# bioinfomaticsCSU/deepsignal

Hardware: AMD Instinct MI355X
Metric: CpG sites/sec (batch=512, k=17, sig=360) (higher is better)
Workload: dtype f32; 1 GPU; configs[1]: 1xMI355X, batch=512, random-init CpG model weights, synthetic (17,360) features, fp32; batch=512, kmer_len=17, signal_len=360

## Files before the change

### deepsignal_amd/csrc/ds_kernels.hip

```cpp
#include "ds_device.h"

namespace ds {


template <int MT, int NT, int WM, int WN, int EPI, int AMODE, int BD, int KS, bool BF = false>
__global__ __launch_bounds__(64 * WM * WN, 1) void gemm_kernel(const GemmLaunch* __restrict__ L)
{
    static_assert(KS == 1, "the in-workgroup K split is retired (profiles/EXPERIMENTS.md)");
    constexpr int BM = WM * MT * 32;
    constexpr int LDA = KC + 4;
    constexpr int NTHR = 64 * WM * WN;
    constexpr int SLOTS = (BM * 4 + NTHR - 1) / NTHR;
    __shared__ __attribute__((aligned(16))) float smem_[2 * BM * LDA];

    const int lane = threadIdx.x & 63, wave_all = __builtin_amdgcn_readfirstlane(threadIdx.x >> 6);
    const int kl = wave_all / (WM * WN);
    const int wave = wave_all % (WM * WN);
    const int tid = threadIdx.x - kl * NTHR;
    float* const As0 = smem_ + kl * BM * LDA;
    float* const As1 = smem_ + (1 + kl) * BM * LDA;
    const int wm = wave % WM, wn = wave / WM;
    int bid;
    {
        const int total = L->total_tiles, q = total >> 3, r = total & 7;
// ... 525 lines not shown
    for (int nt = 0; nt < NT; ++nt) {
        cp[nt] = make_float4(0.f, 0.f, 0.f, 0.f);
        if (!C.c_zero) cp[nt] = gload4(C.c + mt_off + (unsigned)(((ng * 2 + nj) * NT + nt)) * 256 + lane4);
    }

#pragma unroll
    for (int nt = 0; nt < NT; ++nt) {
        asm volatile("" : "+v"(cp[nt].x), "+v"(cp[nt].y), "+v"(cp[nt].z), "+v"(cp[nt].w));
        asm volatile("" : "+v"(acc[nt]));
    }
    DS_LSTAMP(2, __builtin_amdgcn_s_memtime());
    const float* const fa0 = ring + mi * 256 + lane4;
    const float* const fb0 = ring + (2 + nj * NT) * 256 + lane4;
    auto stage = [&](int st, auto slot_c) __attribute__((always_inline)) {
        constexpr int SLOT = decltype(slot_c)::value;
        if (st + 1 < nstages) asm volatile("s_waitcnt vmcnt(%0)" ::"n"(LPS) : "memory");
        else asm volatile("s_waitcnt vmcnt(0)" ::: "memory");
        __builtin_amdgcn_s_barrier();
        if (st + 2 < nstages) request(st + 2, (SLOT + 2) % 3);
#pragma unroll
        for (int kgi = 0; kgi < KGS; ++kgi) {
            const float4 a = *reinterpret_cast<const float4*>(fa0 + SLOT * STAGE + kgi * FR * 256);
#pragma unroll
            for (int nt = 0; nt < NT; ++nt) {
                const float4 b = *reinterpret_cast<const float4*>(fb0 + SLOT * STAGE + (kgi * FR + nt) * 256);
                acc[nt] = __builtin_amdgcn_mfma_f32_32x32x2f32(b.x, a.x, acc[nt], 0, 0, 0);
                acc[nt] = __builtin_amdgcn_mfma_f32_32x32x2f32(b.y, a.y, acc[nt], 0, 0, 0);
                acc[nt] = __builtin_amdgcn_mfma_f32_32x32x2f32(b.z, a.z, acc[nt], 0, 0, 0);
                acc[nt] = __builtin_amdgcn_mfma_f32_32x32x2f32(b.w, a.w, acc[nt], 0, 0, 0);
            }
        }
    };
    for (int st = 0; st < nstages;) {
        stage(st, LdsSlot<0>{}); if (++st >= nstages) break;
        stage(st, LdsSlot<1>{}); if (++st >= nstages) break;
        stage(st, LdsSlot<2>{}); ++st;
    }

    DS_LSTAMP(3, __builtin_amdgcn_s_memtime());
    if (!valid) return;
#pragma unroll
    for (int nt = 0; nt < NT; ++nt) {
        const int ntile = (ng * 2 + nj) * NT + nt;
        float4 cn, hn;
        lstm_gates(acc[nt], cp[nt], cn, hn);
        const size_t off = mt_off + (unsigned)ntile * 256 + lane4;
        const v4f co = {cn.x, cn.y, cn.z, cn.w}, ho = {hn.x, hn.y, hn.z, hn.w};
        *(__attribute__((address_space(1))) v4f*)(C.c + off) = co;
        *(__attribute__((address_space(1))) v4f*)(C.h_out + off) = ho;
        if (C.h_row && row < n)
            *(__attribute__((address_space(1))) v4f*)(C.h_row + (size_t)row * 256 + ntile * 8 + 4 * half) = ho;
    }
    DS_LSTAMP(4, __builtin_amdgcn_s_memtime());
    DS_LSTAMP(5, __builtin_amdgcn_s_memrealtime());
#undef DS_LSTAMP
}

constexpr int LSTM_MT_BYTES_BF16 = 32 * 256 * 2;
template <int MTW, int NTW>
__global__ __launch_bounds__(256, MTW * NTW >= 4 ? 2 : 3) void lstm_cell_bf16_kernel(const LstmLaunch L_)
{
    const LstmLaunch* const Lp = &L_;
    constexpr int FRA = 2 * MTW, FRB = 2 * NTW, FR = FRA + FRB;
    constexpr int KGS = 2;
    constexpr int NF = KGS * FR;
    static_assert(NF % 4 == 0, "fragments of a stage are dealt to four waves");
    constexpr int LPS = NF / 4;
    constexpr int STAGE = NF * 256;
    extern __shared__ __attribute__((aligned(16))) float ring[];

    const int lane = threadIdx.x & 63, wave = __builtin_amdgcn_readfirstlane(threadIdx.x >> 6);
    const int mi = wave & 1, nj = wave >> 1;
    unsigned long long* const sdst = (Lp->dbg && blockIdx.x < DBG_MAX_WGS) ? Lp->dbg + (size_t)blockIdx.x * 8 : nullptr;
    const bool stamp = sdst != nullptr && threadIdx.x == 0;
#define DS_LSTAMP(i, v) do { if (stamp) sdst[i] = (v); } while (0)
    DS_LSTAMP(0, __builtin_amdgcn_s_memrealtime());
    DS_LSTAMP(1, __builtin_amdgcn_s_memtime());
    DS_LSTAMP(6, (unsigned long long)__builtin_amdgcn_s_getreg(63492));
    DS_LSTAMP(7, (unsigned long long)__builtin_amdgcn_s_getreg(63508));
    const int bid = lstm_logical_tile(blockIdx.x, gridDim.x, Lp->cls_tiles[0], Lp->cls_tiles[1]);
    const int mtiles = Lp->mtiles;
    const int mblocks = (mtiles + FRA - 1) / FRA;
    constexpr int NGROUPS = 32 / FRB;
    const int per_cell = mblocks * NGROUPS;
    const int ci = bid / per_cell, rem = bid - ci * per_cell;
    const int ng = rem % NGROUPS, mb = rem / NGROUPS;
    const LstmCell& C = Lp->cell[ci];
    const int half = lane >> 5, r31 = lane & 31;
    const int n = Lp->n, T = Lp->T;
    const unsigned lane16 = (unsigned)lane * 16, lane4 = (unsigned)lane * 4;

    const bool has_x = C.ax != nullptr, has_h = C.ah != nullptr;
    const int KS = (has_x ? 16 : 0) + (has_h ? 16 : 0);
    const int nstages = KS / KGS;
    const char* const a0 = reinterpret_cast<const char*>(has_x ? C.ax : C.ah);
    const long dseg = (has_x && has_h) ? (reinterpret_cast<const char*>(C.ah) - reinterpret_cast<const char*>(C.ax)) - 16 * 1024 : 0;
    const char* src[LPS];
    int kgi_[LPS];
    bool is_a[LPS];
#pragma unroll
    for (int j = 0; j < LPS; ++j) {
        const int q = wave + 4 * j, kgi = q / FR, f = q - kgi * FR;
        kgi_[j] = kgi;
        is_a[j] = f < FRA;
        if (f < FRA) {
            const int m = min(mb * FRA + f, mtiles - 1);
            src[j] = a0 + (size_t)m * LSTM_MT_BYTES_BF16 + (size_t)kgi * 1024;
        } else {
            const int ntile = ng * FRB + (f - FRA);
            src[j] = reinterpret_cast<const char*>(C.Bp) + ((size_t)ntile * C.kg_stride + kgi) * 1024;
        }
    }
    const unsigned ring_lds = (unsigned)(size_t)(__attribute__((address_space(3))) float*)ring;
    auto request = [&](int st, int slot) __attribute__((always_inline)) {
        const unsigned dst = __builtin_amdgcn_readfirstlane(ring_lds + (slot * STAGE + wave * 256) * 4);
#pragma unroll
        for (int j = 0; j < LPS; ++j) {
            const int ks = st * KGS + kgi_[j];
            const long off = (long)st * (KGS * 1024) + ((is_a[j] && ks >= 16) ? dseg : 0);
            glds16s(src[j] + off, lane16, dst + j * 4096);
        }
    };
    if (nstages > 0) request(0, 0);
    if (nstages > 1) request(1, 1);

    int mt[MTW];
    bool valid[MTW];
#pragma unroll
    for (int i = 0; i < MTW; ++i) {
        const int raw = mb * FRA + mi * MTW + i;
        valid[i] = raw < mtiles;
        mt[i] = valid[i] ? raw : mtiles - 1;
    }
    floatx16 acc[MTW][NTW];
    float4 cp[MTW][NTW];
#pragma unroll
    for (int i = 0; i < MTW; ++i) {
        const int row = mt[i] * 32 + r31;
        const int rowc = row < n ? row : n - 1;
#pragma unroll
        for (int j = 0; j < NTW; ++j) lstm_acc_init(C, (ng * FRB + nj * NTW + j) * 8 + 4 * half, rowc, T, acc[i][j]);
    }
    const bool c_zero = C.c_zero != 0;
#pragma unroll
    for (int i = 0; i < MTW; ++i)
#pragma unroll
        for (int j = 0; j < NTW; ++j) {
            cp[i][j] = make_float4(0.f, 0.f, 0.f, 0.f);
            if (!c_zero) cp[i][j] = gload4(C.c + (size_t)mt[i] * LSTM_MT_FLOATS + (unsigned)(ng * FRB + nj * NTW + j) * 256 + lane4);
        }
#pragma unroll
    for (int i = 0; i < MTW; ++i)
#pragma unroll
        for (int j = 0; j < NTW; ++j) {
            asm volatile("" : "+v"(cp[i][j].x), "+v"(cp[i][j].y), "+v"(cp[i][j].z), "+v"(cp[i][j].w));
            asm volatile("" : "+v"(acc[i][j]));
        }
    DS_LSTAMP(2, __builtin_amdgcn_s_memtime());

    const float* const fa0 = ring + (mi * MTW) * 256 + lane4;
    const float* const fb0 = ring + (FRA + nj * NTW) * 256 + lane4;
    auto stage = [&](int st, auto slot_c) __attribute__((always_inline)) {
        constexpr int SLOT = decltype(slot_c)::value;
        if (st + 1 < nstages) asm volatile("s_waitcnt vmcnt(%0)" ::"n"(LPS) : "memory");
        else asm volatile("s_waitcnt vmcnt(0)" ::: "memory");
        __builtin_amdgcn_s_barrier();
        if (st + 2 < nstages) request(st + 2, (SLOT + 2) % 3);
#pragma unroll
        for (int kgi = 0; kgi < KGS; ++kgi) {
            float4 a[MTW], b[NTW];
#pragma unroll
            for (int i = 0; i < MTW; ++i) a[i] = *reinterpret_cast<const float4*>(fa0 + SLOT * STAGE + (kgi * FR + i) * 256);
#pragma unroll
            for (int j = 0; j < NTW; ++j) b[j] = *reinterpret_cast<const float4*>(fb0 + SLOT * STAGE + (kgi * FR + j) * 256);
#pragma unroll
            for (int i = 0; i < MTW; ++i)
#pragma unroll
                for (int j = 0; j < NTW; ++j) acc[i][j] = mfma_bf_early(b[j], a[i], acc[i][j]);
        }
    };
    for (int st = 0; st < nstages;) {
        stage(st, LdsSlot<0>{}); if (++st >= nstages) break;
        stage(st, LdsSlot<1>{}); if (++st >= nstages) break;
        stage(st, LdsSlot<2>{}); ++st;
    }
    DS_LSTAMP(3, __builtin_amdgcn_s_memtime());

    typedef unsigned int u2v __attribute__((ext_vector_type(2)));
#pragma unroll
    for (int i = 0; i < MTW; ++i) {
        if (!valid[i]) continue;
        const int row = mt[i] * 32 + r31;
#pragma unroll
        for (int j = 0; j < NTW; ++j) {
            const int ntile = ng * FRB + nj * NTW + j;
            float4 cn, hn;
            lstm_gates(acc[i][j], cp[i][j], cn, hn);
            const v4f co = {cn.x, cn.y, cn.z, cn.w};
            *(__attribute__((address_space(1))) v4f*)(C.c + (size_t)mt[i] * LSTM_MT_FLOATS + (unsigned)ntile * 256 + lane4) = co;
            const u2v ho = {pack_bf2(hn.x, hn.y), pack_bf2(hn.z, hn.w)};
            char* const hb = reinterpret_cast<char*>(C.h_out) + (size_t)mt[i] * LSTM_MT_BYTES_BF16 + (unsigned)(ntile >> 1) * 1024 +
                             (unsigned)(((ntile & 1) * 32 + r31) * 16 + half * 8);
            *(__attribute__((address_space(1))) u2v*)hb = ho;
            if (C.h_row && row < n) {
                const v4f hr = {hn.x, hn.y, hn.z, hn.w};
                *(__attribute__((address_space(1))) v4f*)(C.h_row + (size_t)row * 256 + ntile * 8 + 4 * half) = hr;
            }
        }
    }
    DS_LSTAMP(4, __builtin_amdgcn_s_memtime());
    DS_LSTAMP(5, __builtin_amdgcn_s_memrealtime());
#undef DS_LSTAMP
}

hipError_t launch_lstm_cells(LstmTile tile, const LstmLaunch& L, hipStream_t s)
{
    if (L.ncell <= 0 || L.mtiles <= 0) return hipSuccess;
    const dim3 grid(L.ncell * lstm_tiles_per_cell(tile, L.mtiles));
    switch (tile) {
    case LT_LDS1: hipLaunchKernelGGL(lstm_cell_lds_kernel<1>, grid, dim3(256), 3 * 1 * 4 * 1024, s, L); break;
    case LT_LDS2: hipLaunchKernelGGL(lstm_cell_lds_kernel<2>, grid, dim3(256), 3 * 2 * 6 * 1024, s, L); break;
    case LT_B11: hipLaunchKernelGGL((lstm_cell_bf16_kernel<1, 1>), grid, dim3(256), 3 * 2 * 4 * 1024, s, L); break;
    case LT_B12: hipLaunchKernelGGL((lstm_cell_bf16_kernel<1, 2>), grid, dim3(256), 3 * 2 * 6 * 1024, s, L); break;
    case LT_B22: hipLaunchKernelGGL((lstm_cell_bf16_kernel<2, 2>), grid, dim3(256), 3 * 2 * 8 * 1024, s, L); break;
    case LT_F1: hipLaunchKernelGGL(lstm_cell_kernel<1>, grid, dim3(256), 0, s, L); break;
    case LT_F4: hipLaunchKernelGGL(lstm_cell_kernel<4>, grid, dim3(256), 0, s, L); break;
    case LT_S11: case LT_S12: case LT_S22: case LT_S28: case LT_COUNT: return hipErrorInvalidValue;
    }
    return hipGetLastError();
}

#ifndef DS_FUSED_WPS
#define DS_FUSED_WPS 2
#endif
#ifndef DS_FUSED_BD
#define DS_FUSED_BD 2
#endif
#ifndef DS_FUSED_POOLPRIO
#define DS_FUSED_POOLPRIO 0
#endif
#ifndef DS_FUSED_VD
#define DS_FUSED_VD 2
#endif
constexpr int F_LDA = KC + 4;
constexpr int F_LD1 = 100;
constexpr int F_LD2 = 68;

size_t inception_fused_lds_bytes(int tm, int W, int spt)
{
    const int tr32 = tm * 32;
    return (size_t)(tr32 * F_LD1 + (spt * (W + 4) + 5) * F_LD1 + tr32 * F_LD2 + tr32 + 192) * sizeof(float);
}

__device__ __forceinline__ void fused_unit_prefetch(const float* __restrict__ Bp, int ntaps, int nt, int lane, float4 (&ub)[20])
{
    const float* bsrc = Bp + ((size_t)(nt * ntaps * 4) * 64 + lane) * 4;
#pragma unroll
    for (int g = 0; g < 20; ++g)
        if (g < ntaps * 4) ub[g] = gload4(bsrc + g * 256);
}

template <int NTAPS>
__device__ __forceinline__ void fused_conv_unit(const float* T1, int rm, int coloff, int lane, const float4 (&ub)[20], floatx16& acc)
{
    const float* base = T1 + rm * F_LD1 + coloff + (lane >> 5) * 4;
#pragma unroll
    for (int t = 0; t < NTAPS; ++t) {
        const float* arow = base + (t - NTAPS / 2) * F_LD1;
#pragma unroll
        for (int g = 0; g < 4; ++g) {
            const float4 a = *reinterpret_cast<const float4*>(arow + g * 8);
            acc = __builtin_amdgcn_mfma_f32_32x32x2f32(ub[t * 4 + g].x, a.x, acc, 0, 0, 0);
            acc = __builtin_amdgcn_mfma_f32_32x32x2f32(ub[t * 4 + g].y, a.y, acc, 0, 0, 0);
            acc = __builtin_amdgcn_mfma_f32_32x32x2f32(ub[t * 4 + g].z, a.z, acc, 0, 0, 0);
            acc = __builtin_amdgcn_mfma_f32_32x32x2f32(ub[t * 4 + g].w, a.w, acc, 0, 0, 0);
        }
    }
}

struct FusedTagT { static constexpr bool value = true; };
struct FusedTagF { static constexpr bool value = false; };

template <int TM>
__device__ __forceinline__ void inception_fused_body(const FusedChain& c)
{
    constexpr int TR32 = TM * 32;
    extern __shared__ __attribute__((aligned(16))) float smem[];
    float* Ad = smem;
    float* Ys = smem;
    float* T1 = smem + TR32 * F_LD1;
    const int W = c.m[0].W, spt = c.m[0].spt;
    float* T2 = T1 + (spt * (W + 4) + 5) * F_LD1;
    int* rowmap = reinterpret_cast<int*>(T2 + TR32 * F_LD2);
    float* const Bs = reinterpret_cast<float*>(rowmap + TR32);
    const int site0 = blockIdx.x * spt;
    const int nhere = min(spt, c.m[0].n_sites - site0);
    const int TRv = nhere * W;
    const size_t grow0 = (size_t)site0 * W;
    for (int i = threadIdx.x; i < (spt * (W + 4) + 5) * (F_LD1 / 4); i += 512)
        reinterpret_cast<float4*>(T1)[i] = make_float4(0.f, 0.f, 0.f, 0.f);
    if (threadIdx.x < TR32)
        rowmap[threadIdx.x] = (int)threadIdx.x < TRv ? ((int)threadIdx.x / W) * (W + 4) + 2 + (int)threadIdx.x % W : spt * (W + 4) + 2;

    for (int mi = 0; mi < c.nmod; ++mi) {
    const FusedArgs& a = c.m[mi];
    int tid_opaque = threadIdx.x, wave_opaque = __builtin_amdgcn_readfirstlane(threadIdx.x >> 6);
    asm volatile("" : "+v"(tid_opaque), "+s"(wave_opaque));
    const int tid = tid_opaque, lane = tid & 63, wave = wave_opaque;
    const int cin = a.cin;
    const gptr1w Yg = (gptr1w)(a.Y + grow0 * 240);

    const bool stamp = a.dbg != nullptr && lane == 0 && (wave == 0 || wave == 7) && blockIdx.x < DBG_MAX_WGS;
#define DS_STAMP(i) do { if (stamp) (a.dbg + ((size_t)blockIdx.x * 2 + (wave == 7)) * 8)[i] = __builtin_amdgcn_s_memtime(); } while (0)
    DS_STAMP(0);
    if (tid >= 256 && tid < 448) {
        const int q = tid - 256;
        Bs[q] = gload((q < 64 ? a.bias5b : q < 128 ? a.bias3b : a.bias4b) + (q & 63));
    }

    const bool stager = tid < TR32 * 4;
    const int sr = tid >> 2, sq = tid & 3;
    const int rr = sr < TRv ? sr : TRv - 1;
    const bool pooled_in = a.pool_win > 0;
    const float *pc, *pq = nullptr, *pr = nullptr;
    if (!pooled_in) {
        pc = a.X + (grow0 + rr) * cin + sq * 4;
    } else {
        const int s_ = rr / W, w_ = rr % W;
        const int i0 = 2 * w_ - a.pool_pad;
        const int ia = i0 < 0 ? i0 + 1 : i0;
        const int ib = i0 + 1 < a.pool_win ? (i0 + 1 < 0 ? ia : i0 + 1) : ia;
        const int ic = i0 + 2 < a.pool_win ? i0 + 2 : ib;
        const float* sb = a.X + ((size_t)(site0 + s_) * a.pool_win) * cin + sq * 4;
        pc = sb + (size_t)ia * cin;
        pq = sb + (size_t)ib * cin;
        pr = sb + (size_t)ic * cin;
    }
    const float* bp = a.Bp1 + ((size_t)wave * ((cin + 31) / 32 * 4) * 64 + lane) * 4;

    const int h4 = 4 * (lane >> 5), rlane = lane & 31;
    floatx16 acc[TM];
    {
        float4 bv[4];
#pragma unroll
        for (int g = 0; g < 4; ++g) {
            bv[g] = gload4(a.bias1 + wave * 32 + 8 * g + h4);
            if (wave < 2) {
                const float4 t = gload4(a.bias5c + wave * 32 + 8 * g + h4);
                bv[g].x += t.x; bv[g].y += t.y; bv[g].z += t.z; bv[g].w += t.w;
            }
        }
#pragma unroll
        for (int mt = 0; mt < TM; ++mt)
#pragma unroll
            for (int g = 0; g < 4; ++g) {
                acc[mt][4 * g + 0] = bv[g].x; acc[mt][4 * g + 1] = bv[g].y;
                acc[mt][4 * g + 2] = bv[g].z; acc[mt][4 * g + 3] = bv[g].w;
            }
    }

    int offm[TM], offp[TM];
#pragma unroll
    for (int mt = 0; mt < TM; ++mt) {
        const int row = mt * 32 + (lane & 31);
        const int w = row % W;
        offm[mt] = (row < TRv && w > 0) ? -F_LDA : 0;
        offp[mt] = (row < TRv && w < W - 1) ? F_LDA : 0;
    }

    const int nchunks = cin / KC;

    __builtin_assume(nchunks >= 15 && nchunks <= 16);
    auto run_p1 = [&](auto pool_tag) {
        constexpr bool POOL = decltype(pool_tag)::value;
        constexpr int VD = DS_FUSED_VD;
        float4 vc[VD];
        constexpr int BD = DS_FUSED_BD;
        float4 bq[BD][2];
        float4 af[2][2][TM];
        auto load_a = [&](int V) __attribute__((always_inline)) {
            if (!POOL && stager) {
                vc[V] = gload4(pc); pc += KC;
                if (pooled_in) {
                    vc[V] = f4max_relu(f4max_relu(vc[V], gload4(pq)), gload4(pr));
                    pq += KC; pr += KC;
                }
            }
        };
        auto store_a = [&](int X, int V) __attribute__((always_inline)) {
            if (!POOL && stager) *reinterpret_cast<float4*>(Ad + X * TR32 * F_LDA + sr * F_LDA + sq * 4) = vc[V];
        };
        auto load_b = [&](int Bi) __attribute__((always_inline)) {
            bq[Bi][0] = gload4(bp);
            bq[Bi][1] = gload4(bp + 256);
            bp += 512;
        };
        auto read_frags = [&](int X) __attribute__((always_inline)) {
#pragma unroll
            for (int rs = 0; rs < 2; ++rs)
#pragma unroll
                for (int mt = 0; mt < TM; ++mt) {
                    const float* q = Ad + X * TR32 * F_LDA + (mt * 32 + (lane & 31)) * F_LDA + rs * 8 + (lane >> 5) * 4;
                    float4 v = *reinterpret_cast<const float4*>(q);
                    if (POOL) v = f4max_relu(f4max_relu(v, *reinterpret_cast<const float4*>(q + offm[mt])), *reinterpret_cast<const float4*>(q + offp[mt]));
                    af[X][rs][mt] = v;
                }
        };
        auto mfma_rs = [&](int X, int Bi, int rs) __attribute__((always_inline)) {
#pragma unroll
            for (int mt = 0; mt < TM; ++mt) {
                acc[mt] = __builtin_amdgcn_mfma_f32_32x32x2f32(bq[Bi][rs].x, af[X][rs][mt].x, acc[mt], 0, 0, 0);
                acc[mt] = __builtin_amdgcn_mfma_f32_32x32x2f32(bq[Bi][rs].y, af[X][rs][mt].y, acc[mt], 0, 0, 0);
                acc[mt] = __builtin_amdgcn_mfma_f32_32x32x2f32(bq[Bi][rs].z, af[X][rs][mt].z, acc[mt], 0, 0, 0);
                acc[mt] = __builtin_amdgcn_mfma_f32_32x32x2f32(bq[Bi][rs].w, af[X][rs][mt].w, acc[mt], 0, 0, 0);
            }
        };
#pragma unroll
        for (int i = 0; i < VD; ++i) load_a(i);
#pragma unroll
        for (int i = 0; i < BD - 1; ++i) load_b(i);
        store_a(0, 0);
        __syncthreads();
        read_frags(0);
#pragma unroll
        for (int c = 0; c < 16; ++c) {
            if (c < nchunks) {
                const int X = c & 1;
                const bool has1 = c + 1 < nchunks;
                if (c + VD < nchunks) load_a(c % VD);
                if (c + BD - 1 < nchunks) load_b((c + BD - 1) % BD);
                if (has1) store_a(X ^ 1, (c + 1) % VD);
                mfma_rs(X, c % BD, 0);
                __builtin_amdgcn_sched_barrier(0);
                __syncthreads();
                if (has1) read_frags(X ^ 1);
                mfma_rs(X, c % BD, 1);
                __builtin_amdgcn_sched_group_barrier(0x8, 1, 0);
                if (has1) __builtin_amdgcn_sched_group_barrier(0x100, (POOL ? 6 : 2) * TM, 0);
                __builtin_amdgcn_sched_group_barrier(0x8, 4 * TM, 0);
                __builtin_amdgcn_sched_barrier(0);
            }
        }
    };
    if (wave >= 6) { __builtin_amdgcn_s_setprio(DS_FUSED_POOLPRIO); run_p1(FusedTagT{}); __builtin_amdgcn_s_setprio(0); }
    else run_p1(FusedTagF{});
    DS_STAMP(1);
    __syncthreads();
    DS_STAMP(2);

    int a1k = 0, a1m = 0, a1n = 0, a2k = 0, a2m = 0, a2n = 0;
    int b1k = 0, b1m = 0, b1n = 0, b2k = 0, b2m = 0, b2n = 0;
    if (TM == 3) {
        if (wave < 6) { a1k = 1; a1m = wave % 3; a1n = wave / 3; }
        else { a1k = 2; a1m = 0; a1n = wave - 6; }
        if (wave >= 2) { b1k = 3; b1m = (wave - 2) % 3; b1n = (wave - 2) / 3; }
        if (wave >= 4) { b2k = 2; b2m = 1 + ((wave - 4) >> 1); b2n = (wave - 4) & 1; }
    } else if (TM == 2) {
        if (wave < 4) { a1k = 1; a1m = wave & 1; a1n = wave >> 1; }
        else { a1k = 2; a1m = wave & 1; a1n = (wave - 4) >> 1; }
        if (wave >= 2 && wave < 6) { b1k = 3; b1m = (wave - 2) & 1; b1n = (wave - 2) >> 1; }
    } else {
        if (wave < 2) { a1k = 1; a1n = wave; }
        else if (wave < 4) { a1k = 2; a1n = wave - 2; }
        else if (wave < 6) { a1k = 3; a1n = wave - 4; }
    }
    auto unit_Bp = [&](int k) { return k == 1 ? a.Bp5b : k == 2 ? a.Bp3b : a.Bp4b; };
    auto unit_taps = [&](int k) { return k == 3 ? 5 : 3; };
    float4 pf[20];
#pragma unroll
    for (int g = 0; g < 20; ++g) pf[g] = make_float4(0.f, 0.f, 0.f, 0.f);
    if (a1k) fused_unit_prefetch(unit_Bp(a1k), unit_taps(a1k), a1n, lane, pf);

    if (wave >= 3 && wave <= 5) {
#pragma unroll
        for (int mt = 0; mt < TM; ++mt) {
            const int rm = rowmap[mt * 32 + rlane];
#pragma unroll
            for (int g = 0; g < 4; ++g)
                *reinterpret_cast<float4*>(T1 + rm * F_LD1 + (wave * 32 - 96) + 8 * g + h4) =
                    make_float4(relu_f(acc[mt][4 * g]), relu_f(acc[mt][4 * g + 1]), relu_f(acc[mt][4 * g + 2]),
                                relu_f(acc[mt][4 * g + 3]));
        }
    } else if (wave != 0) {
#pragma unroll
        for (int g = 0; g < 4; ++g) {
            const int col = wave * 32 + 8 * g + h4;
            if (col >= 48 && col < 240) {
                const int ycol = col < 96 ? col : col - 192;
#pragma unroll
                for (int mt = 0; mt < TM; ++mt)
                    *reinterpret_cast<float4*>(Ys + (mt * 32 + rlane) * F_LD1 + ycol) =
                        make_float4(relu_f(acc[mt][4 * g]), relu_f(acc[mt][4 * g + 1]), relu_f(acc[mt][4 * g + 2]),
                                    relu_f(acc[mt][4 * g + 3]));
            }
        }
    }
    DS_STAMP(3);
    __syncthreads();
    DS_STAMP(4);
    for (int idx = tid; idx < TR32 * 24; idx += 512) {
        const int row = idx / 24, q = idx - row * 24;
        if (row < TRv) {
            const float4 v = *reinterpret_cast<const float4*>(Ys + row * F_LD1 + q * 4);
            v4f o = {v.x, v.y, v.z, v.w};
            *(__attribute__((address_space(1))) v4f*)(Yg + (unsigned)(row * 240 + q * 4)) = o;
        }
    }

    auto run_unit = [&](int kind, int mt, int nt) {
        floatx16 u;
        const float* bsrc = Bs + (kind == 1 ? 0 : kind == 2 ? 64 : 128) + nt * 32 + h4;
#pragma unroll
        for (int g = 0; g < 4; ++g) {
            const float4 t = *reinterpret_cast<const float4*>(bsrc + 8 * g);
            u[4 * g] = t.x; u[4 * g + 1] = t.y; u[4 * g + 2] = t.z; u[4 * g + 3] = t.w;
        }
        const int row = mt * 32 + rlane;
        const int rm = rowmap[row];
        if (kind == 1) {
            fused_conv_unit<3>(T1, rm, 64, lane, pf, u);
#pragma unroll
            for (int g = 0; g < 4; ++g)
                *reinterpret_cast<float4*>(T2 + row * F_LD2 + nt * 32 + 8 * g + h4) =
                    make_float4(relu_f(u[4 * g]), relu_f(u[4 * g + 1]), relu_f(u[4 * g + 2]), relu_f(u[4 * g + 3]));
        } else {
            if (kind == 2) fused_conv_unit<3>(T1, rm, 0, lane, pf, u);
            else fused_conv_unit<5>(T1, rm, 32, lane, pf, u);
            const int ybase = kind == 2 ? 96 : 144;
            if (row < TRv) {
#pragma unroll
                for (int g = 0; g < 4; ++g)
                    if (nt * 32 + 8 * g < 48) {
                        v4f o = {relu_f(u[4 * g]), relu_f(u[4 * g + 1]), relu_f(u[4 * g + 2]), relu_f(u[4 * g + 3])};
                        *(__attribute__((address_space(1))) v4f*)(Yg + (unsigned)(row * 240 + ybase + nt * 32 + 8 * g + h4)) = o;
                    }
            }
        }
    };

    if (a1k) run_unit(a1k, a1m, a1n);
    if (a2k) {
        fused_unit_prefetch(unit_Bp(a2k), unit_taps(a2k), a2n, lane, pf);
        run_unit(a2k, a2m, a2n);
    }
    float4 b5c[8];
#pragma unroll
    for (int g = 0; g < 8; ++g) b5c[g] = make_float4(0.f, 0.f, 0.f, 0.f);
    if (wave < 2) {
#pragma unroll
        for (int g = 0; g < 8; ++g) b5c[g] = gload4(a.Bp5c + ((size_t)(wave * 8 + g) * 64 + lane) * 4);
    } else if (b1k) {
        fused_unit_prefetch(unit_Bp(b1k), unit_taps(b1k), b1n, lane, pf);
    }
    DS_STAMP(5);
    __syncthreads();
    DS_STAMP(6);

    if (wave < 2) {
#pragma unroll
        for (int mt = 0; mt < TM; ++mt) {
            const float* base = T2 + (mt * 32 + rlane) * F_LD2 + h4;
#pragma unroll
            for (int g = 0; g < 8; ++g) {
                const float4 av = *reinterpret_cast<const float4*>(base + g * 8);
                acc[mt] = __builtin_amdgcn_mfma_f32_32x32x2f32(b5c[g].x, av.x, acc[mt], 0, 0, 0);
                acc[mt] = __builtin_amdgcn_mfma_f32_32x32x2f32(b5c[g].y, av.y, acc[mt], 0, 0, 0);
                acc[mt] = __builtin_amdgcn_mfma_f32_32x32x2f32(b5c[g].z, av.z, acc[mt], 0, 0, 0);
                acc[mt] = __builtin_amdgcn_mfma_f32_32x32x2f32(b5c[g].w, av.w, acc[mt], 0, 0, 0);
            }
        }
#pragma unroll
        for (int mt = 0; mt < TM; ++mt) {
            const int row = mt * 32 + rlane;
            if (row < TRv) {
#pragma unroll
                for (int g = 0; g < 4; ++g)
                    if (wave * 32 + 8 * g < 48) {
                        v4f o = {relu_f(acc[mt][4 * g]), relu_f(acc[mt][4 * g + 1]), relu_f(acc[mt][4 * g + 2]),
                                 relu_f(acc[mt][4 * g + 3])};
                        *(__attribute__((address_space(1))) v4f*)(Yg + (unsigned)(row * 240 + 192 + wave * 32 + 8 * g + h4)) = o;
                    }
            }
        }
    } else {
        if (b1k) run_unit(b1k, b1m, b1n);
        if (b2k) {
            fused_unit_prefetch(unit_Bp(b2k), unit_taps(b2k), b2n, lane, pf);
            run_unit(b2k, b2m, b2n);
        }
    }
    DS_STAMP(7);
#undef DS_STAMP
    if (mi + 1 < c.nmod) __syncthreads();
    }
}

template <int TM>
__global__ __launch_bounds__(512, DS_FUSED_WPS) void inception_fused_kernel(const FusedChain c) { inception_fused_body<TM>(c); }
static bool fused_chain_ok(const FusedChain& c)
{
    if (c.nmod <= 0 || c.nmod > FUSED_CHAIN_MAX) return false;
    for (int i = 1; i < c.nmod; ++i)
        if (c.m[i].W != c.m[0].W || c.m[i].spt != c.m[0].spt || c.m[i].n_sites != c.m[0].n_sites || c.m[i].pool_win != 0 ||
            c.m[i].X != c.m[i - 1].Y) return false;
    return true;
}

hipError_t launch_inception_fused(int tm, const FusedChain& c, hipStream_t s)
{
    if (!fused_chain_ok(c)) return hipErrorInvalidValue;
    const FusedArgs& a = c.m[0];
    if (a.n_sites <= 0) return hipSuccess;
    for (int i = 0; i < c.nmod; ++i)
        if (c.m[i].cin != 240 && c.m[i].cin != 256) return hipErrorInvalidValue;
    const size_t lds = inception_fused_lds_bytes(tm, a.W, a.spt);
    const int grid = (a.n_sites + a.spt - 1) / a.spt;
    switch (tm) {
    case 1: hipLaunchKernelGGL(inception_fused_kernel<1>, dim3(grid), dim3(512), lds, s, c); break;
    case 2: hipLaunchKernelGGL(inception_fused_kernel<2>, dim3(grid), dim3(512), lds, s, c); break;
    case 3: hipLaunchKernelGGL(inception_fused_kernel<3>, dim3(grid), dim3(512), lds, s, c); break;
    default: return hipErrorInvalidValue;
    }
    return hipGetLastError();
}

#ifndef DS_FUSEDB_WPS
#define DS_FUSEDB_WPS 4
#endif
#ifndef DS_FUSEDB_POOLPRIO
#define DS_FUSEDB_POOLPRIO 2
#endif
#ifndef DS_FUSEDB_RING
#define DS_FUSEDB_RING 2
#endif
constexpr int B_LDA = 132;
constexpr int B_LD1 = 52;

size_t inception_fused_bf16_lds_bytes(int tm, int W, int spt)
{
    const int tr32 = tm * 32;
    return (size_t)(tr32 * B_LDA + (spt * (W + 4) + 5) * B_LD1 + tr32 + 192) * sizeof(float);
}

__device__ __forceinline__ void fusedb_unit_prefetch(const float* __restrict__ Bp, int ntaps, int nt, int lane, float4 (&ub)[10])
{
    const int ks = (ntaps * 32 + 63) / 64 * 4;
    const float* bsrc = Bp + ((size_t)(nt * ks) * 64 + lane) * 4;
#pragma unroll
    for (int g = 0; g < 10; ++g)
        if (g < ntaps * 2) ub[g] = gload4(bsrc + g * 256);
}

template <int NTAPS>
__device__ __forceinline__ void fusedb_conv_unit(const float* T1, int rm, int coloff_units, int lane, const float4 (&ub)[10], floatx16& acc)
{
    const float* base = T1 + rm * B_LD1 + coloff_units + (lane >> 5) * 4;
#pragma unroll
    for (int t = 0; t < NTAPS; ++t) {
        const float* arow = base + (t - NTAPS / 2) * B_LD1;
#pragma unroll
        for (int j = 0; j < 2; ++j)
            acc = mfma_bf(ub[t * 2 + j], *reinterpret_cast<const float4*>(arow + j * 8), acc);
    }
}

template <int NTAPS, int NM>
__device__ __forceinline__ void fusedb_conv_units(const float* T1, const int (&rm)[NM], int coloff_units, int lane, const float4 (&ub)[10], floatx16 (&acc)[NM])
{
#pragma unroll
    for (int t = 0; t < NTAPS; ++t)
#pragma unroll
        for (int j = 0; j < 2; ++j)
#pragma unroll
            for (int m = 0; m < NM; ++m)
                acc[m] = mfma_bf(ub[t * 2 + j], *reinterpret_cast<const float4*>(T1 + (rm[m] + t - NTAPS / 2) * B_LD1 + coloff_units + (lane >> 5) * 4 + j * 8), acc[m]);
}

template <int TM>
__global__ __launch_bounds__(512, TM >= 2 ? DS_FUSEDB_WPS : 2) void inception_fused_bf16_kernel(const FusedChain c)
{
    constexpr int TR32 = TM * 32;
    extern __shared__ __attribute__((aligned(16))) float smem[];
    float* const As = smem;
    float* const T1 = smem + TR32 * B_LDA;
    const int tid = threadIdx.x, wave = __builtin_amdgcn_readfirstlane(tid >> 6);
    const int W = c.m[0].W, spt = c.m[0].spt, cinu = c.m[0].cin;
    int* const rowmap = reinterpret_cast<int*>(T1 + (spt * (W + 4) + 5) * B_LD1);
    float* const Bs = reinterpret_cast<float*>(rowmap + TR32);
    unsigned short* const T1h = reinterpret_cast<unsigned short*>(T1);
    unsigned short* const Ash = reinterpret_cast<unsigned short*>(As);
    auto lds_barrier = []() __attribute__((always_inline)) { asm volatile("s_waitcnt lgkmcnt(0)\n\ts_barrier" ::: "memory"); };
    constexpr int NSLOT = TR32 * 32 / 512;

    const int site0 = blockIdx.x * spt;
    const int TRv = min(spt, c.m[0].n_sites - site0) * W;
    typedef __attribute__((address_space(1))) unsigned short* gbf16w;

    auto pack4 = [](float x0, float x1, float x2, float x3) -> uint2 {
        return make_uint2(pack_bf2(relu_f(x0), relu_f(x1)), pack_bf2(relu_f(x2), relu_f(x3)));
    };

    int ak = 0, am = 0, an = 0;
    int bk = 0, bm = 0, bn = 0;
    if (TM == 3) {
        if (wave < 6) { ak = 1; am = wave % 3; an = wave / 3; }
        else { ak = 2; am = 0; an = wave - 6; }
        if (wave >= 2) { bk = 3; bm = (wave - 2) % 3; bn = (wave - 2) / 3; }
    } else if (TM == 2) {
        if (wave < 4) { ak = 1; am = wave & 1; an = wave >> 1; }
        else { ak = 2; am = wave & 1; an = (wave - 4) >> 1; }
        if (wave >= 2 && wave < 6) { bk = 3; bm = (wave - 2) & 1; bn = (wave - 2) >> 1; }
    } else {
        if (wave < 2) { ak = 1; an = wave; }
        else if (wave < 4) { ak = 2; an = wave - 2; }
        else if (wave < 6) { ak = 3; an = wave - 4; }
    }

    for (int i = tid; i < (spt * (W + 4) + 5) * (B_LD1 / 4); i += 512)
        reinterpret_cast<float4*>(T1)[i] = make_float4(0.f, 0.f, 0.f, 0.f);
    if (tid < TR32)
        rowmap[tid] = tid < TRv ? (tid / W) * (W + 4) + 2 + tid % W : spt * (W + 4) + 2;

    for (int mi = 0; mi < c.nmod; ++mi) {
    const FusedArgs& a = c.m[mi];
    int tid_opaque = threadIdx.x, wave_opaque = __builtin_amdgcn_readfirstlane(threadIdx.x >> 6);
    asm volatile("" : "+v"(tid_opaque), "+s"(wave_opaque));
    const int tid = tid_opaque, lane = tid & 63, h4 = 4 * (lane >> 5), rlane = lane & 31, wave = wave_opaque;
    const bool stamp = a.dbg != nullptr && lane == 0 && (wave == 0 || wave == 7) && blockIdx.x < DBG_MAX_WGS;
#define DS_STAMP(i) do { if (stamp) (a.dbg + ((size_t)blockIdx.x * 2 + (wave == 7)) * 8)[i] = __builtin_amdgcn_s_memtime(); } while (0)
    DS_STAMP(0);
    auto unit_Bp = [&](int k) { return k == 1 ? a.Bp5b : k == 2 ? a.Bp3b : a.Bp4b; };
    auto unit_taps = [&](int k) { return k == 3 ? 5 : 3; };

    float bsv;
    float4 bv[4], tv[4];
    auto request_biases = [&]() __attribute__((always_inline)) {
        bsv = tid < 192 ? gload((tid < 64 ? a.bias5b : tid < 128 ? a.bias3b : a.bias4b) + (tid & 63)) : 0.0f;
#pragma unroll
        for (int g = 0; g < 4; ++g) {
            bv[g] = gload4(a.bias1 + wave * 32 + 8 * g + h4);
            tv[g] = gload4(a.bias5c + (wave < 2 ? wave : 0) * 32 + 8 * g + h4);
        }
    };
    if (mi == 0) {
        const bool pooled_in = a.pool_win > 0;
        float4 st[NSLOT];
        const size_t grow0 = (size_t)site0 * W;
        if (!pooled_in) {
#pragma unroll
            for (int i = 0; i < NSLOT; ++i) {
                const int id = tid + i * 512, row = id >> 5, q = id & 31;
                const int rr = row < TRv ? row : TRv - 1;
                st[i] = gload4_nt(a.X + (grow0 + rr) * cinu + q * 4);
            }
        } else {
#pragma unroll
            for (int i = 0; i < NSLOT; ++i) {
                const int id = tid + i * 512, row = id >> 5, q = id & 31;
                const int rr = row < TRv ? row : TRv - 1;
                const int s_ = rr / W, w_ = rr % W;
                const int i0 = 2 * w_ - a.pool_pad;
                const int ia = i0 < 0 ? i0 + 1 : i0;
                const int ib = i0 + 1 < a.pool_win ? (i0 + 1 < 0 ? ia : i0 + 1) : ia;
                const int ic = i0 + 2 < a.pool_win ? i0 + 2 : ib;
                const float* sb = a.X + ((size_t)(site0 + s_) * a.pool_win) * cinu + q * 4;
                st[i] = bf8max_relu(bf8max_relu(gload4(sb + (size_t)ia * cinu), gload4(sb + (size_t)ib * cinu)), gload4(sb + (size_t)ic * cinu));
            }
        }
        request_biases();
#pragma unroll
        for (int i = 0; i < NSLOT; ++i) {
            const int id = tid + i * 512, row = id >> 5, q = id & 31;
            *reinterpret_cast<float4*>(As + row * B_LDA + q * 4) = st[i];
        }
    } else {
        request_biases();
    }
    if (tid < 192) Bs[tid] = bsv;
    const char* const bp_base = reinterpret_cast<const char*>(a.Bp1) + (size_t)wave * ((cinu + 31) / 32 * 4) * 1024;
    const unsigned lane16 = (unsigned)lane * 16;
    auto bfrag = [&](int g) __attribute__((always_inline)) { return gload4(reinterpret_cast<const float*>(bp_base + g * 1024 + lane16)); };
    float4 bw[DS_FUSEDB_RING];
#pragma unroll
    for (int g = 0; g < DS_FUSEDB_RING; ++g) bw[g] = bfrag(g);
    floatx16 acc[TM];
    {
        const float tsel = wave < 2 ? 1.0f : 0.0f;
#pragma unroll
        for (int g = 0; g < 4; ++g) {
            const float4 b = make_float4(fmaf(tsel, tv[g].x, bv[g].x), fmaf(tsel, tv[g].y, bv[g].y), fmaf(tsel, tv[g].z, bv[g].z),
                                         fmaf(tsel, tv[g].w, bv[g].w));
#pragma unroll
            for (int mt = 0; mt < TM; ++mt) {
                acc[mt][4 * g + 0] = b.x; acc[mt][4 * g + 1] = b.y;
                acc[mt][4 * g + 2] = b.z; acc[mt][4 * g + 3] = b.w;
            }
        }
    }
    if (mi == 0) lds_barrier();
    DS_STAMP(1);

    auto run_p1 = [&](auto pool_tag) __attribute__((always_inline)) {
        constexpr bool POOL = decltype(pool_tag)::value;
        const float* const src = As + rlane * B_LDA + h4;
        if (!POOL) {
            float4 af[TM];
#pragma unroll
            for (int mt = 0; mt < TM; ++mt) af[mt] = *reinterpret_cast<const float4*>(src + mt * 32 * B_LDA);
#pragma unroll
            for (int g = 0; g < 16; ++g) {
#pragma unroll
                for (int mt = 0; mt < TM; ++mt) acc[mt] = mfma_bf(bw[g % DS_FUSEDB_RING], af[mt], acc[mt]);
                if (g + DS_FUSEDB_RING < 16) bw[g % DS_FUSEDB_RING] = bfrag(g + DS_FUSEDB_RING);
                if (g + 1 < 16) {
#pragma unroll
                    for (int mt = 0; mt < TM; ++mt) af[mt] = *reinterpret_cast<const float4*>(src + mt * 32 * B_LDA + (g + 1) * 8);
                }
                __builtin_amdgcn_sched_barrier(0);
            }
        } else {
            int om[TM], op[TM];
#pragma unroll
            for (int mt = 0; mt < TM; ++mt) {
                const int row = mt * 32 + rlane, w = row % W;
                om[mt] = (row < TRv && w > 0) ? -B_LDA : 0;
                op[mt] = (row < TRv && w < W - 1) ? B_LDA : 0;
            }
            float4 raw[TM][3];
#pragma unroll
            for (int mt = 0; mt < TM; ++mt) {
                const float* q = src + mt * 32 * B_LDA;
                raw[mt][0] = *reinterpret_cast<const float4*>(q);
                raw[mt][1] = *reinterpret_cast<const float4*>(q + om[mt]);
                raw[mt][2] = *reinterpret_cast<const float4*>(q + op[mt]);
            }
#pragma unroll
            for (int g = 0; g < 16; ++g) {
#pragma unroll
                for (int mt = 0; mt < TM; ++mt) {
                    const float4 af = bf8max_relu(bf8max_relu(raw[mt][0], raw[mt][1]), raw[mt][2]);
                    if (g + 1 < 16) {
                        const float* q = src + mt * 32 * B_LDA + (g + 1) * 8;
                        raw[mt][0] = *reinterpret_cast<const float4*>(q);
                        raw[mt][1] = *reinterpret_cast<const float4*>(q + om[mt]);
                        raw[mt][2] = *reinterpret_cast<const float4*>(q + op[mt]);
                    }
                    acc[mt] = mfma_bf(bw[g % DS_FUSEDB_RING], af, acc[mt]);
                }
                if (g + DS_FUSEDB_RING < 16) bw[g % DS_FUSEDB_RING] = bfrag(g + DS_FUSEDB_RING);
                __builtin_amdgcn_sched_barrier(0);
            }
        }
    };
    if (wave >= 6) { __builtin_amdgcn_s_setprio(DS_FUSEDB_POOLPRIO); run_p1(FusedTagT{}); __builtin_amdgcn_s_setprio(0); }
    else run_p1(FusedTagF{});
    DS_STAMP(2);
    lds_barrier();
    float4 pf[10];
#pragma unroll
    for (int g = 6; g < 10; ++g) pf[g] = make_float4(0.f, 0.f, 0.f, 0.f);
    if (ak) fusedb_unit_prefetch(unit_Bp(ak), unit_taps(ak), an, lane, pf);

    if (wave >= 3 && wave <= 5) {
#pragma unroll
        for (int mt = 0; mt < TM; ++mt) {
            const int rm = rowmap[mt * 32 + rlane];
#pragma unroll
            for (int g = 0; g < 4; ++g)
                *reinterpret_cast<uint2*>(T1h + rm * (2 * B_LD1) + (wave * 32 - 96) + 8 * g + h4) =
                    pack4(acc[mt][4 * g], acc[mt][4 * g + 1], acc[mt][4 * g + 2], acc[mt][4 * g + 3]);
        }
    } else if (wave != 0) {
#pragma unroll
        for (int g = 0; g < 4; ++g) {
            const int col = wave * 32 + 8 * g + h4;
            if (col >= 48 && col < 240) {
                const int ycol = col < 96 ? col : col - 192;
#pragma unroll
                for (int mt = 0; mt < TM; ++mt)
                    *reinterpret_cast<uint2*>(Ash + (mt * 32 + rlane) * (2 * B_LDA) + ycol) =
                        pack4(acc[mt][4 * g], acc[mt][4 * g + 1], acc[mt][4 * g + 2], acc[mt][4 * g + 3]);
            }
        }
    }
    lds_barrier();
    DS_STAMP(3);

    auto run_unit = [&](int kind, int mt, int nt) __attribute__((always_inline)) {
        floatx16 u;
        const float* bsrc = Bs + (kind == 1 ? 0 : kind == 2 ? 64 : 128) + nt * 32 + h4;
#pragma unroll
        for (int g = 0; g < 4; ++g) {
            const float4 t = *reinterpret_cast<const float4*>(bsrc + 8 * g);
            u[4 * g] = t.x; u[4 * g + 1] = t.y; u[4 * g + 2] = t.z; u[4 * g + 3] = t.w;
        }
        const int row = mt * 32 + rlane;
// ... 831 lines not shown
```

Measured before the change: 420,300 sites/s.

## Prefetch next module's biases and first weight fragments before module barrier

In the fused inception chain kernel, the per-module bias loads (bias1, bias5c, branch biases) and the first BD-1 weight fragments are now issued into registers before the inter-module __syncthreads, via a request_start helper. The following module consumes these registers instead of issuing fresh global loads at its start. This hides global-load latency behind the barrier and the previous module's tail. In exchange it keeps extra registers live across modules, which could add register pressure or spills, and it adds a sched_barrier before the second unit.

```diff
diff --git a/deepsignal_amd/csrc/ds_kernels.hip b/deepsignal_amd/csrc/ds_kernels.hip
--- a/deepsignal_amd/csrc/ds_kernels.hip
+++ b/deepsignal_amd/csrc/ds_kernels.hip
@@ -851,6 +851,26 @@
     if (threadIdx.x < TR32)
         rowmap[threadIdx.x] = (int)threadIdx.x < TRv ? ((int)threadIdx.x / W) * (W + 4) + 2 + (int)threadIdx.x % W : spt * (W + 4) + 2;
 
+    static_assert(DS_FUSED_BD >= 2, "the weight fragments of chunk 0 travel across the module boundary");
+    float4 nbv[4], nb5[4], nbq[DS_FUSED_BD - 1][2];
+    float nbs;
+    auto request_start = [&](const FusedArgs& n, int wave, int lane) __attribute__((always_inline)) {
+        const float* nbp = n.Bp1 + ((size_t)wave * ((n.cin + 31) / 32 * 4) * 64 + lane) * 4;
+#pragma unroll
+        for (int g = 0; g < 4; ++g) {
+            nbv[g] = gload4(n.bias1 + wave * 32 + 8 * g + 4 * (lane >> 5));
+            nb5[g] = gload4(n.bias5c + (wave < 2 ? wave : 0) * 32 + 8 * g + 4 * (lane >> 5));
+        }
+#pragma unroll
+        for (int i = 0; i < DS_FUSED_BD - 1; ++i) {
+            nbq[i][0] = gload4(nbp + i * 512);
+            nbq[i][1] = gload4(nbp + i * 512 + 256);
+        }
+        nbs = 0.f;
+        if (wave >= 4 && wave < 7) nbs = gload((wave == 4 ? n.bias5b : wave == 5 ? n.bias3b : n.bias4b) + lane);
+    };
+    request_start(c.m[0], __builtin_amdgcn_readfirstlane(threadIdx.x >> 6), threadIdx.x & 63);
+
     for (int mi = 0; mi < c.nmod; ++mi) {
     const FusedArgs& a = c.m[mi];
     int tid_opaque = threadIdx.x, wave_opaque = __builtin_amdgcn_readfirstlane(threadIdx.x >> 6);
@@ -862,10 +882,7 @@
     const bool stamp = a.dbg != nullptr && lane == 0 && (wave == 0 || wave == 7) && blockIdx.x < DBG_MAX_WGS;
 #define DS_STAMP(i) do { if (stamp) (a.dbg + ((size_t)blockIdx.x * 2 + (wave == 7)) * 8)[i] = __builtin_amdgcn_s_memtime(); } while (0)
     DS_STAMP(0);
-    if (tid >= 256 && tid < 448) {
-        const int q = tid - 256;
-        Bs[q] = gload((q < 64 ? a.bias5b : q < 128 ? a.bias3b : a.bias4b) + (q & 63));
-    }
+    if (wave >= 4 && wave < 7) Bs[tid - 256] = nbs;
 
     const bool stager = tid < TR32 * 4;
     const int sr = tid >> 2, sq = tid & 3;
@@ -885,7 +902,7 @@
         pq = sb + (size_t)ib * cin;
         pr = sb + (size_t)ic * cin;
     }
-    const float* bp = a.Bp1 + ((size_t)wave * ((cin + 31) / 32 * 4) * 64 + lane) * 4;
+    const float* bp = a.Bp1 + ((size_t)wave * ((cin + 31) / 32 * 4) * 64 + lane) * 4 + (DS_FUSED_BD - 1) * 512;
 
     const int h4 = 4 * (lane >> 5), rlane = lane & 31;
     floatx16 acc[TM];
@@ -893,9 +910,9 @@
         float4 bv[4];
 #pragma unroll
         for (int g = 0; g < 4; ++g) {
-            bv[g] = gload4(a.bias1 + wave * 32 + 8 * g + h4);
+            bv[g] = nbv[g];
             if (wave < 2) {
-                const float4 t = gload4(a.bias5c + wave * 32 + 8 * g + h4);
+                const float4 t = nb5[g];
                 bv[g].x += t.x; bv[g].y += t.y; bv[g].z += t.z; bv[g].w += t.w;
             }
         }
@@ -967,7 +984,7 @@
 #pragma unroll
         for (int i = 0; i < VD; ++i) load_a(i);
 #pragma unroll
-        for (int i = 0; i < BD - 1; ++i) load_b(i);
+        for (int i = 0; i < BD - 1; ++i) { bq[i][0] = nbq[i][0]; bq[i][1] = nbq[i][1]; }
         store_a(0, 0);
         __syncthreads();
         read_frags(0);
@@ -1135,12 +1152,16 @@
         if (b1k) run_unit(b1k, b1m, b1n);
         if (b2k) {
             fused_unit_prefetch(unit_Bp(b2k), unit_taps(b2k), b2n, lane, pf);
+            __builtin_amdgcn_sched_barrier(0);
             run_unit(b2k, b2m, b2n);
         }
     }
     DS_STAMP(7);
 #undef DS_STAMP
-    if (mi + 1 < c.nmod) __syncthreads();
+    if (mi + 1 < c.nmod) {
+        request_start(c.m[mi + 1], wave, lane);
+        __syncthreads();
+    }
     }
 }
 
```

Result: no change. 420,700 sites/s, median of 4 (+0.1%).
